# DavidPetrus/ood_object_detection

Hardware: AMD Instinct MI355X
Metric: images/sec, tf_efficientdet_d0 640px bf16 inference + OOD score (DetBenchPredict end-to-end) (higher is better)
Workload: dtype bf16; 1 GPU; tf_efficientdet_d0 640x640 batch=64/GPU C=90, DetBenchPredict: backbone+BiFPN+heads+OOD energy/max-logit+top-k(5000)+decode+hard NMS; global_batch=64, parallelism=image-sharded dp1, no collective, weights=seeded reference init, randomised BN stats, class bias 0, launch=hipgraph, images_in_flight=192

## Files before the change

### ood_object_detection_amd/csrc/common.h

```cpp
#pragma once
#include <hip/hip_runtime.h>
#include <stdint.h>
#include "../../include/effdet_hip.h"

#define EFFDET_OK 0
#define EFFDET_EINVAL (-22)
#define EFFDET_ELAUNCH (-5)

typedef __bf16 bf16_t;
typedef __bf16 bf16x8 __attribute__((ext_vector_type(8)));
typedef float f32x4 __attribute__((ext_vector_type(4)));
typedef unsigned int u32x4 __attribute__((ext_vector_type(4)));

#define DEV __device__ __forceinline__

#define EFFDET_ENTER() (void)hipGetLastError()

extern thread_local int effdet_last_hip_error;
#define EFFDET_DEVICE_ERROR_CODE 0x7EFFDE7
__attribute__((visibility("hidden"))) extern volatile int* effdet_err_host;
__attribute__((visibility("hidden"))) int* effdet_device_error_word();
static inline int effdet_check_launch() {
    hipError_t e = hipGetLastError();
    if (e != hipSuccess) { effdet_last_hip_error = (int)e; return EFFDET_ELAUNCH; }
// ... 7 lines not shown
DEV float fast_silu(float x) { return x * __builtin_amdgcn_rcpf(1.0f + fast_exp(-x)); }
DEV float sigmoid_train(float x) { return __builtin_amdgcn_rcpf(1.0f + __builtin_amdgcn_exp2f(x * -1.4426950408889634f)); }
DEV float silu_train(float x) { return x * sigmoid_train(x); }
DEV float silu_grad(float z) { const float s = sigmoid_train(z); return s * (1.0f + z * (1.0f - s)); }

struct bf16p_t;
template <typename T> struct FastMath { static constexpr bool value = sizeof(T) == 2; };
template <> struct FastMath<bf16p_t> { static constexpr bool value = true; };
template <typename T> DEV float silu_t(float x) {
    if constexpr (FastMath<T>::value) return fast_silu(x); else return silu_f(x);
}
template <typename T> DEV float exp_t(float x) {
    if constexpr (FastMath<T>::value) return fast_exp(x); else return expf(x);
}

typedef float f32x2 __attribute__((ext_vector_type(2)));
DEV f32x4 silu4_scaled(const f32x4 t, const float addc) {
    const f32x2 t0 = {t[0], t[1]}, t1 = {t[2], t[3]};
    const float d00 = __builtin_amdgcn_exp2f(t0[0]) + addc, d01 = __builtin_amdgcn_exp2f(t0[1]) + addc;
    const float d10 = __builtin_amdgcn_exp2f(t1[0]) + addc, d11 = __builtin_amdgcn_exp2f(t1[1]) + addc;
    const f32x2 y0 = t0 * f32x2{__builtin_amdgcn_rcpf(d00), __builtin_amdgcn_rcpf(d01)};
    const f32x2 y1 = t1 * f32x2{__builtin_amdgcn_rcpf(d10), __builtin_amdgcn_rcpf(d11)};
    return f32x4{y0[0], y0[1], y1[0], y1[1]};
}

DEV f32x4 silu4_fast(const f32x4 x) {
    const f32x2 x0 = {x[0], x[1]}, x1 = {x[2], x[3]};
    const f32x2 t0 = x0 * -1.4426950408889634f, t1 = x1 * -1.4426950408889634f;
    const f32x2 d0 = f32x2{__builtin_amdgcn_exp2f(t0[0]), __builtin_amdgcn_exp2f(t0[1])} + 1.0f;
    const f32x2 d1 = f32x2{__builtin_amdgcn_exp2f(t1[0]), __builtin_amdgcn_exp2f(t1[1])} + 1.0f;
    const f32x2 y0 = x0 * f32x2{__builtin_amdgcn_rcpf(d0[0]), __builtin_amdgcn_rcpf(d0[1])};
    const f32x2 y1 = x1 * f32x2{__builtin_amdgcn_rcpf(d1[0]), __builtin_amdgcn_rcpf(d1[1])};
    return f32x4{y0[0], y0[1], y1[0], y1[1]};
}

template <int V> struct IntC { static constexpr int value = V; };

template <typename T> DEV f32x4 bn_silu4(const f32x4 acc, const f32x4 sc, const f32x4 sh) {
    if constexpr (FastMath<T>::value) {
        const f32x2 x0 = f32x2{acc[0], acc[1]} * f32x2{sc[0], sc[1]} + f32x2{sh[0], sh[1]};
        const f32x2 x1 = f32x2{acc[2], acc[3]} * f32x2{sc[2], sc[3]} + f32x2{sh[2], sh[3]};
        const f32x2 t0 = x0 * -1.4426950408889634f, t1 = x1 * -1.4426950408889634f;
        const f32x2 d0 = f32x2{__builtin_amdgcn_exp2f(t0[0]), __builtin_amdgcn_exp2f(t0[1])} + 1.0f;
        const f32x2 d1 = f32x2{__builtin_amdgcn_exp2f(t1[0]), __builtin_amdgcn_exp2f(t1[1])} + 1.0f;
        const f32x2 y0 = x0 * f32x2{__builtin_amdgcn_rcpf(d0[0]), __builtin_amdgcn_rcpf(d0[1])};
        const f32x2 y1 = x1 * f32x2{__builtin_amdgcn_rcpf(d1[0]), __builtin_amdgcn_rcpf(d1[1])};
        return f32x4{y0[0], y0[1], y1[0], y1[1]};
    } else {
        f32x4 y;
#pragma unroll
        for (int r = 0; r < 4; ++r) y[r] = silu_f(acc[r] * sc[r] + sh[r]);
        return y;
    }
}

template <typename T> struct VecTraits;
template <> struct VecTraits<float> { static constexpr int EPC = 4; };
template <> struct VecTraits<bf16_t> { static constexpr int EPC = 8; };

struct F8 { float v[8]; };

template <typename T> DEV F8 load8(const T* p);
template <> DEV F8 load8<float>(const float* p) {
    F8 r;
    const f32x4 a = *reinterpret_cast<const f32x4*>(p);
    const f32x4 b = *reinterpret_cast<const f32x4*>(p + 4);
// ... 211 lines not shown
```

### ood_object_detection_amd/csrc/sepconv.hip

```cpp
#include "common.h"
#include <type_traits>

namespace {

struct SepInput {
    const void* ptr; long long image_stride;
    int H, W; int mode;
    int pad_t, pad_l;
};
struct SepLevel {
    int H, W, tiles_x, tiles_y, tile_begin, affine_row;
    SepInput in[3];
    void* out; long long out_image_stride;
    long long ood_off;
    int in_affine_row;
    void* dw_out; long long dw_out_image_stride;
};
struct SepArgs {
    int nlevels; SepLevel lv[5];
    int n_in, fuse_mode;
    float fw[3]; float fden;
    float fwn[3];
    int vec_ok;
    int out_f32;
    int pre_act, post_act;
    const float* dw_w;
    const void* pw_w;
    const float* scale; const float* shift;
    int F, N;
    int ood_classes, num_anchors;
    float* ood_energy; float* ood_maxlogit; long long ood_image_stride;
    const float* in_scale; const float* in_shift;
    float* stat_partial;
    int tiles_total;
};

constexpr int FC = 64;



template <typename T> struct Raw8 { u32x4 v[sizeof(T) == 2 ? 1 : 2]; };
template <typename T> DEV Raw8<T> load_raw8(const T* p) {
    Raw8<T> r;
    r.v[0] = *reinterpret_cast<const u32x4*>(p);
    if constexpr (sizeof(T) == 4) r.v[1] = *(reinterpret_cast<const u32x4*>(p) + 1);
    return r;
}
template <typename T> DEV F8 unpack8(const Raw8<T>& r) {
    F8 o;
    if constexpr (IsPair<T>::value) {
        return pair_join8(r.v[0], r.v[1]);
    } else if constexpr (sizeof(T) == 2) {
        const bf16x8 a = __builtin_bit_cast(bf16x8, r.v[0]);
#pragma unroll
        for (int e = 0; e < 8; ++e) o.v[e] = (float)a[e];
    } else {
        const f32x4 a = __builtin_bit_cast(f32x4, r.v[0]), b = __builtin_bit_cast(f32x4, r.v[1]);
#pragma unroll
        for (int e = 0; e < 4; ++e) { o.v[e] = a[e]; o.v[4 + e] = b[e]; }
    }
    return o;
}
template <typename T> DEV Raw8<T> pack8(const F8& f) {
    Raw8<T> r;
    if constexpr (IsPair<T>::value) {
        pair_split8(f, r.v[0], r.v[1]);
    } else if constexpr (sizeof(T) == 2) {
        bf16x8 a;
#pragma unroll
        for (int e = 0; e < 8; ++e) a[e] = (bf16_t)f.v[e];
        r.v[0] = __builtin_bit_cast(u32x4, a);
    } else {
        r.v[0] = __builtin_bit_cast(u32x4, f32x4{f.v[0], f.v[1], f.v[2], f.v[3]});
        r.v[1] = __builtin_bit_cast(u32x4, f32x4{f.v[4], f.v[5], f.v[6], f.v[7]});
    }
    return r;
}

template <typename T>
DEV Raw8<T> fetch_input(const T* base, const SepInput& in, int y, int x, int F, int c) {
    if (in.mode != 2) {
        const int sh = in.mode == 1 ? 1 : 0;
        return load_raw8<T>(base + ((y >> sh) * in.W + (x >> sh)) * F + c);
    }
    F8 m = f8_fill(-INFINITY);
#pragma unroll
    for (int ky = 0; ky < 3; ++ky) {
        const int iy = 2 * y + ky - in.pad_t;
        const int iyc = iy < 0 ? 0 : (iy >= in.H ? in.H - 1 : iy);
#pragma unroll
        for (int kx = 0; kx < 3; ++kx) {
            const int ix = 2 * x + kx - in.pad_l;
            const int ixc = ix < 0 ? 0 : (ix >= in.W ? in.W - 1 : ix);
            const F8 v = load8<T>(base + (iyc * in.W + ixc) * F + c);
            const bool inside = iy == iyc && ix == ixc;
#pragma unroll
            for (int e = 0; e < 8; ++e) m.v[e] = fmaxf(m.v[e], inside ? v.v[e] : -INFINITY);
        }
    }
    return pack8<T>(m);
}

template <typename T>
DEV void store_piece(T* dst, const float (&v)[8], int nvalid, bool vec_ok) {
    if constexpr (IsPair<T>::value) {
        typedef unsigned u32x4_a4 __attribute__((ext_vector_type(4), aligned(4)));
        F8 f;
#pragma unroll
        for (int e = 0; e < 8; ++e) f.v[e] = v[e];
        u32x4 hi, lo;
        pair_split8(f, hi, lo);
        if (nvalid >= 8) {
            *reinterpret_cast<u32x4_a4*>(dst) = hi;
            *(reinterpret_cast<u32x4_a4*>(dst) + 1) = lo;
        }
    } else
    if (vec_ok && nvalid >= 8) {
        if constexpr (sizeof(T) == 2) {
            typedef unsigned u32x4_a4 __attribute__((ext_vector_type(4), aligned(4)));
            bf16x8 a;
#pragma unroll
            for (int e = 0; e < 8; ++e) a[e] = (bf16_t)v[e];
            *reinterpret_cast<u32x4_a4*>(dst) = __builtin_bit_cast(u32x4, a);
        } else {
            typedef float f32x4_a4 __attribute__((ext_vector_type(4), aligned(4)));
            *reinterpret_cast<f32x4_a4*>(dst) = f32x4{v[0], v[1], v[2], v[3]};
            *reinterpret_cast<f32x4_a4*>(dst + 4) = f32x4{v[4], v[5], v[6], v[7]};
        }
    } else {
        if constexpr (!IsPair<T>::value) {
#pragma unroll
            for (int e = 0; e < 8; ++e)
                if (e < nvalid) dst[e] = from_f<T>(v[e]);
        }
    }
}

template <typename T, int TH, int TW, int BN, bool OOD, int NTH, int FT, bool META = false, int NIN = 3, bool BST = false>
__global__ __launch_bounds__(NTH, NTH == 512 ? (FT == 64 && !OOD && !META && !IsPair<T>::value ? 8 : 4) : 2) void sepconv_kernel(SepArgs p) {
    constexpr int BM = TH * TW;
    constexpr int HW_ = (TH + 2) * (TW + 2);
    constexpr int NWAVE = NTH / 64;
    constexpr int WPT = BM / (16 * NWAVE);
    constexpr int NT = BN / 16;
    constexpr int NP = NT / 2;
    static_assert(NT % 2 == 0 && WPT >= 1, "tile shape");
    extern __shared__ __attribute__((aligned(16))) char lds[];

    const int F = FT ? FT : p.F, N = p.N;
    const int fbytes = F * (int)sizeof(T);
    constexpr int PB = OpGeom<T>::PIECE, CHB = OpGeom<T>::CHUNK;
    const int nkc = (fbytes + CHB - 1) / CHB;
    const int arow = nkc * CHB + 16;
    constexpr bool MF = IsFast<T>::value && TW == 16 && NTH == 512;
    constexpr int HROW = FC + (MF ? 16 / (int)sizeof(T) : 0);
    constexpr int HALO_BYTES = HW_ * HROW * (int)sizeof(T);
    constexpr bool CP = MF && FT == 64 && !META;
    const int r0 = CP ? (HALO_BYTES > (BM + BN) * arow ? HALO_BYTES : (BM + BN) * arow)
                      : (HALO_BYTES > BN * arow ? HALO_BYTES : BN * arow);
    char* halo = lds;
    char* Wt = CP ? lds + BM * arow : lds;
    char* At = CP ? lds : lds + r0;
    float* dww = reinterpret_cast<float*>(CP ? lds + r0 : At + BM * arow);
    float* cs = dww + 9 * F;

    const int tid = threadIdx.x, lane = tid & 63, wave = tid >> 6;
    const int b = blockIdx.y;
    int li = 0;
#pragma unroll
    for (int q = 1; q < 5; ++q) if (q < p.nlevels && (int)blockIdx.x >= p.lv[q].tile_begin) li = q;
    const SepLevel& L = p.lv[li];
    const int t = blockIdx.x - L.tile_begin;
    const int y0 = (t / L.tiles_x) * TH, x0 = (t % L.tiles_x) * TW;
    const int H = L.H, W = L.W;

    constexpr int DPC = (9 * 128 + NTH - 1) / NTH;
    const bool d_pref = 9 * F <= DPC * NTH;
    float dpre[DPC];
#pragma unroll
    for (int q = 0; q < DPC; ++q) {
        const int i = tid + NTH * q;
        dpre[q] = (d_pref && i < 9 * F) ? p.dw_w[i] : 0.f;
    }
    if (nkc * CHB > fbytes) {
        const int padb = nkc * CHB - fbytes;
        for (int i = tid; i < BM * (padb / 16); i += NTH) {
            const int row = i / (padb / 16), piece = i % (padb / 16);
            *reinterpret_cast<u32x4*>(At + row * arow + fbytes + piece * 16) = u32x4{0u, 0u, 0u, 0u};
        }
    }
    const T* ib[3];
#pragma unroll
    for (int i = 0; i < 3; ++i) {
        const int ii = i < p.n_in ? i : 0;
        ib[i] = reinterpret_cast<const T*>(L.in[ii].ptr) + (long long)b * L.in[ii].image_stride;
    }
    float fwm[3];
#pragma unroll
    for (int i = 0; i < 3; ++i) fwm[i] = i < p.n_in ? ((IsFast<T>::value && p.fuse_mode == 1) ? p.fwn[i] : p.fw[i]) : 0.f;
    const bool divide = !IsFast<T>::value && p.fuse_mode == 1;

    for (int fc0 = 0; fc0 < F; fc0 += FC) {
        const int fcn = (F - fc0) < FC ? (F - fc0) : FC;
        const int fcg = fcn / 8;
        __syncthreads();
        constexpr int HU = NTH == 512 ? ((FT == 64 && !OOD && !META && NIN > 1) ? 1 : ((FT == 0 && NIN > 1) ? 2 : 3)) : 2;
        for (int it0 = tid; it0 < HW_ * fcg; it0 += HU * NTH) {
            Raw8<T> xin[HU][NIN];
            unsigned okm[HU];
#pragma unroll
            for (int u = 0; u < HU; ++u) {
                const int it_ = it0 + NTH * u;
                const int it = it_ < HW_ * fcg ? it_ : HW_ * fcg - 1;
                const int cgh = it % fcg, hp = it / fcg;
                const int y = y0 + hp / (TW + 2) - 1, x = x0 + hp % (TW + 2) - 1;
                const int yc = y < 0 ? 0 : (y >= H ? H - 1 : y), xc = x < 0 ? 0 : (x >= W ? W - 1 : x);
                okm[u] = (it_ < HW_ * fcg && y == yc && x == xc) ? 0xFFFFFFFFu : 0u;
                const int c = fc0 + cgh * 8;
#pragma unroll
                for (int i = 0; i < NIN; ++i) xin[u][i] = fetch_input<T>(ib[i], L.in[i < p.n_in ? i : 0], yc, xc, F, c);
            }
#pragma unroll
            for (int u = 0; u < HU; ++u) {
                const int it = it0 + NTH * u;
                const int cgh = it % fcg, hp = it / fcg;
                const u32x4 km = {okm[u], okm[u], okm[u], okm[u]};
                F8 v = f8_zero();
                {
                    if (p.fuse_mode == 0) {
                        Raw8<T> r0 = xin[u][0];
                        r0.v[0] = r0.v[0] & km;
                        if constexpr (sizeof(T) == 4) r0.v[1] = r0.v[1] & km;
                        v = unpack8<T>(r0);
                    } else {
#pragma unroll
                        for (int i = 0; i < NIN; ++i) {
                            Raw8<T> ri = xin[u][i];
                            ri.v[0] = ri.v[0] & km;
                            if constexpr (sizeof(T) == 4) ri.v[1] = ri.v[1] & km;
                            const F8 xi = unpack8<T>(ri);
                            if (divide) {
#pragma unroll
                                for (int e = 0; e < 8; ++e) v.v[e] += (xi.v[e] * fwm[i]) / p.fden;
                            } else {
#pragma unroll
                                for (int e = 0; e < 8; ++e) v.v[e] = fmaf(xi.v[e], fwm[i], v.v[e]);
                            }
                        }
                    }
                    if constexpr (META) {
                        if (p.in_scale != nullptr) {
                            const F8 is = load8<float>(p.in_scale + (long long)L.in_affine_row * F + fc0 + cgh * 8);
                            const F8 it = load8<float>(p.in_shift + (long long)L.in_affine_row * F + fc0 + cgh * 8);
#pragma unroll
                            for (int e = 0; e < 8; ++e) v.v[e] = okm[u] ? v.v[e] * is.v[e] + it.v[e] : 0.f;
                        }
                    }
                    if (p.pre_act) {
#pragma unroll
                        for (int e = 0; e < 8; ++e) v.v[e] = silu_t<T>(v.v[e]);
                    }
                }
                if (it < HW_ * fcg) store8<T>(reinterpret_cast<T*>(halo) + hp * HROW + cgh * 8, v);
            }
        }
        if (fc0 == 0) {
            if (d_pref) {
#pragma unroll
                for (int q = 0; q < DPC; ++q) {
                    const int i = tid + NTH * q;
                    if (i < 9 * F) dww[i] = dpre[q];
                }
            } else {
                for (int i = tid; i < 9 * F; i += NTH) dww[i] = p.dw_w[i];
            }
        }
        __syncthreads();
        if constexpr (MF) {
            const int frow_ = lane & 15, fp_ = lane >> 4;
            const int j = wave & 3, part = wave >> 2;
            f32x4 keep[CP ? TH / 2 : 1];
            if (16 * j < fcn) {
                const int hi = fp_ >> 1;
                const bool active = (fp_ & 1) == (frow_ >> 3);
                const int dq = (frow_ & 7) >> 1;
                Frag<T> afr[5];
#pragma unroll
                for (int pr = 0; pr < 5; ++pr) {
                    const int t = 2 * pr + hi;
                    const bool on = active && t < 9 && 16 * j + frow_ < fcn;
                    const float wv = on ? dww[(t < 9 ? t : 0) * F + fc0 + 16 * j + frow_] : 0.f;
                    const bf16_t wh = (bf16_t)wv;
                    const unsigned bits = (unsigned)__builtin_bit_cast(unsigned short, wh) << (16 * (frow_ & 1));
// ... 95 lines not shown
            cpre_s = scale ? scale[n_begin + tc] : 1.0f;
            return;
        }
#pragma unroll
        for (int q = 0; q < WPC; ++q) {
            const int i = tid + NTH * q;
            u32x4 v = {0u, 0u, 0u, 0u};
            if (i < BN * ppr) {
                const int co = i / ppr, piece = i % ppr;
                if (co < n_count && piece * 16 < fbytes)
                    v = *reinterpret_cast<const u32x4*>(reinterpret_cast<const char*>(p.pw_w) +
                                                        (long long)(n_begin + co) * fbytes + piece * 16);
            }
            wpre[q] = v;
        }
        if (tid < BN) {
            cpre_s = (scale && tid < n_count) ? scale[n_begin + tid] : 1.0f;
            cpre_t = tid < n_count ? shift[n_begin + tid] : 0.0f;
        }
    };
    if (prefetch) w_fetch(0);

    int pix_off[WPT];
    bool pix_in[WPT];
#pragma unroll
    for (int i = 0; i < WPT; ++i) {
        const int prow = 16 * WPT * wave + 16 * i + frow;
        const int y = y0 + prow / TW, x = x0 + prow % TW;
        pix_in[i] = y < H && x < W;
        pix_off[i] = (y * W + x) * N;
    }
    __amdgpu_buffer_rsrc_t ors, ers, mrs;
    constexpr int OB = IsPair<T>::value ? 4 : 2;
    if constexpr (BST) {
        ors = __builtin_amdgcn_make_buffer_rsrc(reinterpret_cast<char*>(L.out) + (long long)b * L.out_image_stride * OB, 0, H * W * N * OB, 0x00020000);
        ers = __builtin_amdgcn_make_buffer_rsrc(reinterpret_cast<char*>(p.ood_energy + (long long)b * p.ood_image_stride + L.ood_off), 0,
                                                H * W * p.num_anchors * 4, 0x00020000);
        mrs = __builtin_amdgcn_make_buffer_rsrc(reinterpret_cast<char*>(p.ood_maxlogit + (long long)b * p.ood_image_stride + L.ood_off), 0,
                                                H * W * p.num_anchors * 4, 0x00020000);
    }
    int o128[BST ? WPT : 1][NP], otail[BST ? WPT : 1][3], oscore[BST ? WPT : 1];
    const int jstar = C / 32;
    if constexpr (BST) {
        constexpr int OOB = 0x7FFFFFF0;
#pragma unroll
        for (int i = 0; i < WPT; ++i) {
            const int sb = pix_off[i] * OB + fpiece * 8 * OB;
#pragma unroll
            for (int J = 0; J < NP; ++J) o128[i][J] = (pix_in[i] && C - (32 * J + 8 * fpiece) >= 8) ? sb + 32 * OB * J : OOB;
            const int nvt = C - (32 * jstar + 8 * fpiece);
#pragma unroll
            for (int d = 0; d < 3; ++d)
                otail[i][d] = (pix_in[i] && nvt > 0 && nvt < 8 && 2 * d < nvt) ? sb + 32 * OB * jstar + 2 * OB * d : OOB;
            oscore[i] = (pix_in[i] && fpiece == 0) ? (pix_off[i] / N) * p.num_anchors * 4 : OOB;
        }
    }
    float run_m[WPT], run_s[WPT];
    constexpr float LOG2E = 1.4426950408889634f;

    for (int ch = 0; ch < nchunks; ++ch) {
        int n_begin, n_count;
        chunk_range(ch, n_begin, n_count);
        __syncthreads();
        if constexpr (META) {
            if (ch == 0 && L.dw_out != nullptr) {
                T* dwo = reinterpret_cast<T*>(L.dw_out) + (long long)b * L.dw_out_image_stride;
// ... 10 lines not shown
        if (BST) {
#pragma unroll
            for (int q = 0; q < WPC; ++q) {
                const int i = tid + NTH * q < BN * ppr ? tid + NTH * q : BN * ppr - 1;
                const int co = i / ppr, piece = i % ppr;
                const unsigned keep = (co < n_count && piece * 16 < fbytes) ? 0xFFFFFFFFu : 0u;
                *reinterpret_cast<u32x4*>(Wt + lds_row(co) * arow + piece * 16) = wpre[q] & u32x4{keep, keep, keep, keep};
            }
            if (tid < BN) cs[BN + tid] = tid < n_count ? cpre_t : -INFINITY;
        } else if (prefetch) {
#pragma unroll
            for (int q = 0; q < WPC; ++q) {
                const int i = tid + NTH * q;
                if (i < BN * ppr) *reinterpret_cast<u32x4*>(Wt + lds_row(i / ppr) * arow + (i % ppr) * 16) = wpre[q];
            }
            if (tid < BN) { cs[tid] = cpre_s; cs[BN + tid] = cpre_t; }
        } else {
            for (int i = tid; i < BN * ppr; i += NTH) {
                const int co = i / ppr, piece = i % ppr;
                u32x4 v = {0u, 0u, 0u, 0u};
                if (co < n_count && piece * 16 < fbytes)
                    v = *reinterpret_cast<const u32x4*>(reinterpret_cast<const char*>(p.pw_w) +
                                                        (long long)(n_begin + co) * fbytes + piece * 16);
                *reinterpret_cast<u32x4*>(Wt + lds_row(co) * arow + piece * 16) = v;
            }
            if (tid < BN) {
                cs[tid] = (scale && tid < n_count) ? scale[n_begin + tid] : 1.0f;
                cs[BN + tid] = tid < n_count ? shift[n_begin + tid] : 0.0f;
            }
        }
        __syncthreads();
        if (prefetch && ch + 1 < nchunks) w_fetch(ch + 1);

        const int njp = (n_count + 31) / 32;
        f32x4 acc[WPT][NT];
#pragma unroll
        for (int i = 0; i < WPT; ++i)
#pragma unroll
            for (int j = 0; j < NT; ++j) acc[i][j] = f32x4{0.f, 0.f, 0.f, 0.f};
        for (int kc = 0; kc < nkc; ++kc) {
            Frag<T> xb[WPT];
#pragma unroll
            for (int i = 0; i < WPT; ++i)
                xb[i] = ld_frag<T>(At + (16 * WPT * wave + 16 * i + frow) * arow + kc * CHB + fpiece * PB);
#pragma unroll
            for (int j = 0; j < NT; ++j) {
                if (j < 2 * njp) {
                    const Frag<T> wf = ld_frag<T>(Wt + (16 * j + frow) * arow + kc * CHB + fpiece * PB);
#pragma unroll
                    for (int i = 0; i < WPT; ++i) mma_chunk(wf, xb[i], acc[i][j]);
                }
            }
        }

        if constexpr (BST) {
            constexpr float LN2 = 0.6931471805599453f;
            const int so = n_begin * OB, sa = ch * 4;
#pragma unroll
            for (int i = 0; i < WPT; ++i) {
                f32x4 v[NT];
#pragma unroll
                for (int J = 0; J < NP; ++J) {
                    const int cb = 32 * J + 8 * fpiece;
                    v[2 * J] = acc[i][2 * J] + *reinterpret_cast<const f32x4*>(cs + BN + cb);
                    v[2 * J + 1] = acc[i][2 * J + 1] + *reinterpret_cast<const f32x4*>(cs + BN + cb + 4);
                }
                if constexpr (IsPair<T>::value) {
// ... 12 lines not shown
                    u32x4 pk[NP];
#pragma unroll
                    for (int J = 0; J < NP; ++J) {
                        const bf16x8 a8 = {(bf16_t)v[2 * J][0], (bf16_t)v[2 * J][1], (bf16_t)v[2 * J][2], (bf16_t)v[2 * J][3],
                                           (bf16_t)v[2 * J + 1][0], (bf16_t)v[2 * J + 1][1], (bf16_t)v[2 * J + 1][2], (bf16_t)v[2 * J + 1][3]};
                        pk[J] = __builtin_bit_cast(u32x4, a8);
                        __builtin_amdgcn_raw_buffer_store_b128(pk[J], ors, o128[i][J], so, 0);
                    }
                    u32x4 pt = pk[0];
#pragma unroll
                    for (int J = 1; J < NP; ++J) pt = jstar == J ? pk[J] : pt;
#pragma unroll
                    for (int d = 0; d < 3; ++d) __builtin_amdgcn_raw_buffer_store_b32(pt[d], ors, otail[i][d], so, 0);
                }
                float m = -INFINITY;
#pragma unroll
                for (int j = 0; j < NT; ++j) m = fmaxf(m, fmaxf(fmaxf(v[j][0], v[j][1]), fmaxf(v[j][2], v[j][3])));
                m = fmaxf(m, __shfl_xor(m, 16, 64));
                m = fmaxf(m, __shfl_xor(m, 32, 64));
                const float tl = m * LOG2E;
                f32x2 s2 = {0.f, 0.f};
#pragma unroll
                for (int j = 0; j < NT; ++j) {
                    const f32x2 e0 = f32x2{v[j][0], v[j][1]} * LOG2E - tl, e1 = f32x2{v[j][2], v[j][3]} * LOG2E - tl;
                    s2 += f32x2{__builtin_amdgcn_exp2f(e0[0]), __builtin_amdgcn_exp2f(e0[1])};
                    s2 += f32x2{__builtin_amdgcn_exp2f(e1[0]), __builtin_amdgcn_exp2f(e1[1])};
                }
                float ssum = s2[0] + s2[1];
                ssum += __shfl_xor(ssum, 16, 64);
                ssum += __shfl_xor(ssum, 32, 64);
                const float energy = IsPair<T>::value ? -(m + logf(ssum)) : -(m + LN2 * __builtin_amdgcn_logf(ssum));
                __builtin_amdgcn_raw_buffer_store_b32(__builtin_bit_cast(unsigned, energy), ers, oscore[i], sa, 0);
                __builtin_amdgcn_raw_buffer_store_b32(__builtin_bit_cast(unsigned, m), mrs, oscore[i], sa, 0);
            }
            continue;
        }
        float stq[META ? WPT : 1][META ? NP : 1][8];
        if constexpr (META) {
#pragma unroll
            for (int i = 0; i < WPT; ++i)
#pragma unroll
                for (int J = 0; J < NP; ++J)
#pragma unroll
                    for (int e = 0; e < 8; ++e) stq[i][J][e] = 0.f;
        }
#pragma unroll
        for (int i = 0; i < WPT; ++i) {
            float m = -INFINITY, ssum = 0.f;
            float vals[NP][8];
#pragma unroll
            for (int J = 0; J < NP; ++J) {
                if (J < njp) {
                    const int cb = 32 * J + 8 * fpiece;
                    const f32x4 t0 = *reinterpret_cast<const f32x4*>(cs + BN + cb);
                    const f32x4 t1 = *reinterpret_cast<const f32x4*>(cs + BN + cb + 4);
                    f32x4 s0 = {1.f, 1.f, 1.f, 1.f}, s1 = {1.f, 1.f, 1.f, 1.f};
                    if (scale) {
                        s0 = *reinterpret_cast<const f32x4*>(cs + cb);
                        s1 = *reinterpret_cast<const f32x4*>(cs + cb + 4);
                    }
#pragma unroll
                    for (int r = 0; r < 4; ++r) {
                        float a0 = fmaf(acc[i][2 * J][r], s0[r], t0[r]);
                        float a1 = fmaf(acc[i][2 * J + 1][r], s1[r], t1[r]);
                        if (p.post_act) { a0 = silu_t<T>(a0); a1 = silu_t<T>(a1); }
                        vals[J][r] = a0; vals[J][4 + r] = a1;
// ... 108 lines not shown
                        for (int o = 1; o < 16; o <<= 1) { a += __shfl_xor(a, o, 64); q += __shfl_xor(q, o, 64); }
                        if (frow == 0) { sst[(wave * 2 + 0) * BN + 32 * J + 8 * fpiece + e] = a; sst[(wave * 2 + 1) * BN + 32 * J + 8 * fpiece + e] = q; }
                    }
                __syncthreads();
                if (tid < 2 * BN) {
                    const int which = tid / BN, n = tid % BN;
                    float tot = 0.f;
                    for (int w = 0; w < NWAVE; ++w) tot += sst[(w * 2 + which) * BN + n];
                    if (n < n_count) {
                        float* row = p.stat_partial + (((long long)b * p.tiles_total + blockIdx.x) * 3) * N + n_begin + n;
                        row[(1 + which) * (long long)N] = tot;
                        if (which == 0) row[0] = piv[n];
                    }
                }
            }
        }
    }
}

template <typename T, int TH, int TW, int BN>
size_t sep_lds_bytes(int F, bool cp = false) {
    constexpr int BM = TH * TW;
    constexpr int HW_ = (TH + 2) * (TW + 2);
    const int nkc = (F * (int)sizeof(T) + OpGeom<T>::CHUNK - 1) / OpGeom<T>::CHUNK;
    const int arow = nkc * OpGeom<T>::CHUNK + 16;
    const size_t halo = (size_t)HW_ * (FC + (IsFast<T>::value && TW == 16 ? 16 / (int)sizeof(T) : 0)) * sizeof(T);
    const size_t wt = (size_t)BN * arow;
    if (cp) return (halo > wt + (size_t)BM * arow ? halo : wt + (size_t)BM * arow) + (size_t)9 * F * 4 + (size_t)2 * BN * 4;
    return (halo > wt ? halo : wt) + (size_t)BM * arow + (size_t)9 * F * 4 + (size_t)2 * BN * 4;
}

struct SepPlan { int v[EFFDET_SEPCONV_PLAN_INTS]; };

template <typename T, int TH, int TW, int BN, bool OOD, int NTH, int FT, bool META = false, int NIN = 3, bool BST = false>
int launch_sep(hipStream_t st, SepArgs& a, int B, SepPlan* plan = nullptr) {
    int tiles = 0;
    for (int i = 0; i < a.nlevels; ++i) {
        a.lv[i].tiles_x = (a.lv[i].W + TW - 1) / TW;
        a.lv[i].tiles_y = (a.lv[i].H + TH - 1) / TH;
        a.lv[i].tile_begin = tiles;
        tiles += a.lv[i].tiles_x * a.lv[i].tiles_y;
    }
    const size_t lds = sep_lds_bytes<T, TH, TW, BN>(a.F, IsFast<T>::value && TW == 16 && NTH == 512 && FT == 64 && !META) + (META ? (size_t)(NTH / 64) * 2 * BN * 4 : 0);
    if (lds > 160 * 1024) return EFFDET_EINVAL;
    a.tiles_total = tiles;
    if (plan) {
        constexpr int DPC = (9 * 128 + NTH - 1) / NTH, CHB = OpGeom<T>::CHUNK;
        constexpr int WPC = (BN * (CHB / 8) + NTH - 1) / NTH;
        const int nkc = (a.F * (int)sizeof(T) + CHB - 1) / CHB, ppr = nkc * (CHB / 16);
        const int subs = OOD ? (a.ood_classes + BN - 1) / BN : 1;
        const int v[EFFDET_SEPCONV_PLAN_INTS] = {
            IsPair<T>::value ? 2 : (sizeof(T) == 2 ? 1 : 0), TH, TW, NTH, FT, BN, OOD ? 1 : 0, BST ? 1 : 0, NIN, META ? 1 : 0,
            subs, OOD ? a.num_anchors * subs : (a.N + BN - 1) / BN, tiles, (int)lds,
            9 * a.F <= DPC * NTH ? 1 : 0, BN * ppr <= NTH * WPC ? 1 : 0, a.out_f32, a.vec_ok};
        for (int i = 0; i < EFFDET_SEPCONV_PLAN_INTS; ++i) plan->v[i] = v[i];
        return EFFDET_OK;
    }
    auto kern = sepconv_kernel<T, TH, TW, BN, OOD, NTH, FT, META, NIN, BST>;
    if (lds > 64 * 1024) {
        static bool attr_done = false;
        if (!attr_done) {
            if (hipFuncSetAttribute(reinterpret_cast<const void*>(kern), hipFuncAttributeMaxDynamicSharedMemorySize, 160 * 1024) != hipSuccess)
                return EFFDET_ELAUNCH;
            attr_done = true;
        }
    }
    hipLaunchKernelGGL(kern, dim3(tiles, B), dim3(NTH), lds, st, a);
    return effdet_check_launch();
}

constexpr int BST_TH = 8;
template <typename T, int TH, int TW, int NTH, int FT>
int dispatch_sep_f(hipStream_t st, SepArgs& a, int B, SepPlan* plan = nullptr) {
    if (a.ood_classes > 0) {
        if constexpr (FT == 0) {
            if (sep_lds_bytes<T, TH, TW, 96>(a.F) > 160 * 1024) return launch_sep<T, TH, TW, 64, true, NTH, FT>(st, a, B, plan);
        }
        if constexpr (IsPair<T>::value && NTH == 512) {
            if (a.out_f32 && a.ood_classes % 2 == 0 && a.ood_classes <= 96 && a.F <= 64 && a.scale == nullptr && !a.post_act)
                return launch_sep<T, BST_TH, TW, 96, true, NTH, FT, false, 3, true>(st, a, B, plan);
        }
        if constexpr (sizeof(T) == 2 && NTH == 512) {
            if (a.vec_ok && !a.out_f32 && a.ood_classes % 2 == 0 && a.ood_classes <= 96 && a.F <= 64 && a.scale == nullptr && !a.post_act)
                return launch_sep<T, BST_TH, TW, 96, true, NTH, FT, false, 3, true>(st, a, B, plan);
        }
        return launch_sep<T, TH, TW, 96, true, NTH, FT>(st, a, B, plan);
    }
    if (FT == 64 && a.n_in == 1) return launch_sep<T, TH, TW, 64, false, NTH, FT, false, 1>(st, a, B, plan);
    return launch_sep<T, TH, TW, 64, false, NTH, FT>(st, a, B, plan);
}

template <typename T, int TH, int TW, int NTH>
int dispatch_sep(hipStream_t st, SepArgs& a, int B, SepPlan* plan = nullptr) {
    switch (a.F) {
        case 64:  return dispatch_sep_f<T, TH, TW, NTH, 64>(st, a, B, plan);
        case 88:  return dispatch_sep_f<T, TH, TW, NTH, 88>(st, a, B, plan);
        case 112: return dispatch_sep_f<T, TH, TW, NTH, 112>(st, a, B, plan);
        case 160: return dispatch_sep_f<T, TH, TW, NTH, 160>(st, a, B, plan);
        case 224: return dispatch_sep_f<T, TH, TW, NTH, 224>(st, a, B, plan);
        default:  return dispatch_sep_f<T, TH, TW, NTH, 0>(st, a, B, plan);
    }
}

template <int FT>
int dispatch_sep_pair_8x8(hipStream_t st, SepArgs& a, int B, SepPlan* plan = nullptr) {
    if (a.ood_classes > 0) {
        if constexpr (FT == 0) {
            if (sep_lds_bytes<bf16p_t, 8, 8, 96>(a.F) > 160 * 1024) return launch_sep<bf16p_t, 8, 8, 64, true, 256, 0>(st, a, B, plan);
        }
        return launch_sep<bf16p_t, 8, 8, 96, true, 256, FT>(st, a, B, plan);
    }
    return launch_sep<bf16p_t, 8, 8, 64, false, 256, FT>(st, a, B, plan);
}

}

namespace {
struct MetaExtra {
    const float* in_scale; const float* in_shift; const int* in_affine_row;
// ... 41 lines not shown
    const int* level_hw,
    int n_in,
    const void* const* in_ptr,
    const long long* in_image_stride,
    const int* in_hw,
    const int* in_mode,
    int fuse_mode, const float* fuse_w, float fuse_den, int pre_act,
    const float* dw_w, const void* pw_w, const float* scale, const float* shift,
    const int* affine_row,
    int post_act, int F, int N,
    void* const* out_ptr, const long long* out_image_stride,
    int ood_classes, int num_anchors, float* ood_energy, float* ood_maxlogit,
    long long ood_image_stride, const long long* ood_level_off) {
    if (!level_hw || !in_ptr || !in_image_stride || !in_hw || !in_mode || !dw_w || !pw_w || !shift || !affine_row ||
        !out_ptr || !out_image_stride) return EFFDET_EINVAL;
    const int sym = take_pad_flag(dtype);
    int out_f32 = 0;
    if (sep_check_shape(dtype, out_f32, meta != nullptr, B, nlevels, level_hw, n_in, fuse_mode, F, N, ood_classes, num_anchors) != EFFDET_OK)
        return EFFDET_EINVAL;
    if (fuse_mode != 0 && !fuse_w) return EFFDET_EINVAL;
    if (ood_classes > 0 && (!ood_energy || !ood_maxlogit || !ood_level_off)) return EFFDET_EINVAL;
    SepArgs a;
    a.nlevels = nlevels; a.n_in = n_in; a.fuse_mode = fuse_mode; a.fden = fuse_den;
    for (int i = 0; i < 3; ++i) a.fw[i] = (fuse_mode != 0 && i < n_in) ? fuse_w[i] : 0.f;
    for (int i = 0; i < 3; ++i) a.fwn[i] = fuse_mode == 1 ? a.fw[i] / fuse_den : a.fw[i];
    const size_t esz = (dtype == 0 || out_f32) ? 4 : 2;
    a.out_f32 = out_f32;
    a.vec_ok = sep_rows_dword_aligned(N, ood_classes, esz);
    a.pre_act = pre_act; a.post_act = post_act; a.dw_w = dw_w; a.pw_w = pw_w; a.scale = scale; a.shift = shift;
    a.F = F; a.N = N; a.ood_classes = ood_classes > 0 ? ood_classes : 0; a.num_anchors = num_anchors;
    a.ood_energy = ood_energy; a.ood_maxlogit = ood_maxlogit; a.ood_image_stride = ood_image_stride;
    a.in_scale = meta ? meta->in_scale : nullptr; a.in_shift = meta ? meta->in_shift : nullptr;
    a.stat_partial = meta ? meta->stat_partial : nullptr; a.tiles_total = 0;
    if (meta && ((meta->in_scale != nullptr) != (meta->in_shift != nullptr) || (meta->in_scale && !meta->in_affine_row))) return EFFDET_EINVAL;
    for (int l = 0; l < nlevels; ++l) {
        SepLevel& L = a.lv[l];
        L.in_affine_row = (meta && meta->in_affine_row) ? meta->in_affine_row[l] : 0;
        L.dw_out = (meta && meta->dw_out) ? meta->dw_out[l] : nullptr;
        L.dw_out_image_stride = (meta && meta->dw_out_image_stride) ? meta->dw_out_image_stride[l] : 0;
        if (L.dw_out && reinterpret_cast<uintptr_t>(L.dw_out) % 16) return EFFDET_EINVAL;
        L.H = level_hw[2 * l]; L.W = level_hw[2 * l + 1];
        L.affine_row = affine_row[l];
        L.out = out_ptr[l]; L.out_image_stride = out_image_stride[l];
        L.ood_off = (ood_classes > 0) ? ood_level_off[l] : 0;
        if (!L.out) return EFFDET_EINVAL;
        if (reinterpret_cast<uintptr_t>(L.out) % 16 || ((size_t)L.out_image_stride * esz) % 4) a.vec_ok = 0;
        for (int i = 0; i < n_in; ++i) {
            SepInput& I = L.in[i];
            I.ptr = in_ptr[l * n_in + i]; I.image_stride = in_image_stride[l * n_in + i];
            I.H = in_hw[(l * n_in + i) * 2]; I.W = in_hw[(l * n_in + i) * 2 + 1];
            I.mode = in_mode[l * n_in + i];
            I.pad_t = I.pad_l = 0;
            if (!I.ptr) return EFFDET_EINVAL;
            if (I.mode == 0) { if (I.H != L.H || I.W != L.W) return EFFDET_EINVAL; }
            else if (I.mode == 1) { if (I.H * 2 != L.H || I.W * 2 != L.W) return EFFDET_EINVAL; }
            else if (I.mode == 2) {
                if (same_out(I.H, 2) != L.H || same_out(I.W, 2) != L.W) return EFFDET_EINVAL;
                I.pad_t = pad_before(I.H, 3, 2, sym); I.pad_l = pad_before(I.W, 3, 2, sym);
            } else return EFFDET_EINVAL;
        }
    }
    if (dtype == 2) {
        for (int l = 0; l < nlevels; ++l) {
            if (!out_f32 && (reinterpret_cast<uintptr_t>(a.lv[l].out) % 16 || a.lv[l].out_image_stride % 4)) return EFFDET_EINVAL;
            for (int i = 0; i < n_in; ++i)
                if (reinterpret_cast<uintptr_t>(a.lv[l].in[i].ptr) % 16 || a.lv[l].in[i].image_stride % 4) return EFFDET_EINVAL;
        }
    }
    return sep_dispatch(meta != nullptr, dtype, reinterpret_cast<hipStream_t>(stream), a, B, nullptr);
}

extern "C" int effdet_sepconv_fused(
    void* stream, int dtype, int B, int nlevels, const int* level_hw, int n_in,
    const void* const* in_ptr, const long long* in_image_stride, const int* in_hw, const int* in_mode,
    int fuse_mode, const float* fuse_w, float fuse_den, int pre_act,
    const float* dw_w, const void* pw_w, const float* scale, const float* shift, const int* affine_row,
    int post_act, int F, int N, void* const* out_ptr, const long long* out_image_stride,
    int ood_classes, int num_anchors, float* ood_energy, float* ood_maxlogit,
    long long ood_image_stride, const long long* ood_level_off) {
    EFFDET_ENTER();
    return sepconv_common(nullptr, stream, dtype, B, nlevels, level_hw, n_in, in_ptr, in_image_stride, in_hw, in_mode,
                          fuse_mode, fuse_w, fuse_den, pre_act, dw_w, pw_w, scale, shift, affine_row, post_act, F, N,
                          out_ptr, out_image_stride, ood_classes, num_anchors, ood_energy, ood_maxlogit, ood_image_stride, ood_level_off);
}

extern "C" int effdet_sepconv_meta(
    void* stream, int dtype, int B, int nlevels, const int* level_hw,
    const void* const* in_ptr, const long long* in_image_stride,
    const float* in_scale, const float* in_shift, const int* in_affine_row, int pre_act,
    const float* dw_w, const void* pw_w, const float* bias, int F, int N,
    void* const* out_ptr, const long long* out_image_stride,
    float* stat_partial, void* const* dw_out, const long long* dw_out_image_stride) {
    EFFDET_ENTER();
// ... 101 lines not shown
```

Measured before the change: 17130 images/sec.

## Add trimmed sepconv kernel variants specialised by live inputs and epilogue

Adds TRIM template variants of the bf16 F=64 separable-conv kernel. They load only the live fused inputs, copy raw halo data when there is a single input with no fusion or pre-activation, and skip the max-pool bounds masking when the padding geometry makes it unnecessary. A simplified epilogue applies BN (optionally followed by SiLU) and writes bf16x8 with buffer stores over fixed 64-wide N tiles. The host checks which pooling and padding cases are safe and dispatches to these variants. The aim is fewer registers, less halo-building ALU work and a cheaper store path, at the cost of more template instantiations and correctness that depends on the padding checks.

```diff
diff --git a/ood_object_detection_amd/csrc/common.h b/ood_object_detection_amd/csrc/common.h
--- a/ood_object_detection_amd/csrc/common.h
+++ b/ood_object_detection_amd/csrc/common.h
@@ -63,6 +63,13 @@
     const f32x2 y0 = x0 * f32x2{__builtin_amdgcn_rcpf(d0[0]), __builtin_amdgcn_rcpf(d0[1])};
     const f32x2 y1 = x1 * f32x2{__builtin_amdgcn_rcpf(d1[0]), __builtin_amdgcn_rcpf(d1[1])};
     return f32x4{y0[0], y0[1], y1[0], y1[1]};
+}
+
+DEV f32x2 fma2(const f32x2 a, const f32x2 b, const f32x2 c) { return __builtin_elementwise_fma(a, b, c); }
+DEV f32x4 fma4(const f32x4 a, const f32x4 b, const f32x4 c) {
+    const f32x2 r0 = fma2(f32x2{a[0], a[1]}, f32x2{b[0], b[1]}, f32x2{c[0], c[1]});
+    const f32x2 r1 = fma2(f32x2{a[2], a[3]}, f32x2{b[2], b[3]}, f32x2{c[2], c[3]});
+    return f32x4{r0[0], r0[1], r1[0], r1[1]};
 }
 
 template <int V> struct IntC { static constexpr int value = V; };
diff --git a/ood_object_detection_amd/csrc/sepconv.hip b/ood_object_detection_amd/csrc/sepconv.hip
--- a/ood_object_detection_amd/csrc/sepconv.hip
+++ b/ood_object_detection_amd/csrc/sepconv.hip
@@ -33,6 +33,7 @@
     const float* in_scale; const float* in_shift;
     float* stat_partial;
     int tiles_total;
+    int trim_ok;
 };
 
 constexpr int FC = 64;
@@ -77,9 +78,9 @@
     return r;
 }
 
-template <typename T>
+template <typename T, int POOL = 0>
 DEV Raw8<T> fetch_input(const T* base, const SepInput& in, int y, int x, int F, int c) {
-    if (in.mode != 2) {
+    if (POOL == 2 || in.mode != 2) {
         const int sh = in.mode == 1 ? 1 : 0;
         return load_raw8<T>(base + ((y >> sh) * in.W + (x >> sh)) * F + c);
     }
@@ -93,7 +94,7 @@
             const int ix = 2 * x + kx - in.pad_l;
             const int ixc = ix < 0 ? 0 : (ix >= in.W ? in.W - 1 : ix);
             const F8 v = load8<T>(base + (iyc * in.W + ixc) * F + c);
-            const bool inside = iy == iyc && ix == ixc;
+            const bool inside = POOL == 1 || (iy == iyc && ix == ixc);
 #pragma unroll
             for (int e = 0; e < 8; ++e) m.v[e] = fmaxf(m.v[e], inside ? v.v[e] : -INFINITY);
         }
@@ -136,7 +137,8 @@
     }
 }
 
-template <typename T, int TH, int TW, int BN, bool OOD, int NTH, int FT, bool META = false, int NIN = 3, bool BST = false>
+constexpr int TRIM_RAWH = 4, TRIM_SLE = 8, TRIM_POST = 16, TRIM_DIRECT = 32;
+template <typename T, int TH, int TW, int BN, bool OOD, int NTH, int FT, bool META = false, int NIN = 3, bool BST = false, int TRIM = 0>
 __global__ __launch_bounds__(NTH, NTH == 512 ? (FT == 64 && !OOD && !META && !IsPair<T>::value ? 8 : 4) : 2) void sepconv_kernel(SepArgs p) {
     constexpr int BM = TH * TW;
     constexpr int HW_ = (TH + 2) * (TW + 2);
@@ -145,6 +147,10 @@
     constexpr int NT = BN / 16;
     constexpr int NP = NT / 2;
     static_assert(NT % 2 == 0 && WPT >= 1, "tile shape");
+    constexpr int LIVE = TRIM ? (TRIM & 3) : NIN;
+    constexpr bool PK = TRIM != 0, RAWH = (TRIM & TRIM_RAWH) != 0, SLE = (TRIM & TRIM_SLE) != 0, POST = (TRIM & TRIM_POST) != 0;
+    static_assert(!TRIM || (sizeof(T) == 2 && !IsPair<T>::value && FT == 64 && NTH == 512 && !META), "TRIM forms: bf16, F = 64");
+    static_assert(LIVE >= 1 && LIVE <= NIN && (!RAWH || LIVE == 1) && (!SLE || BN == 64) && (!POST || SLE) && (!TRIM || !OOD), "TRIM bits");
     extern __shared__ __attribute__((aligned(16))) char lds[];
 
     const int F = FT ? FT : p.F, N = p.N;
@@ -189,15 +195,15 @@
             *reinterpret_cast<u32x4*>(At + row * arow + fbytes + piece * 16) = u32x4{0u, 0u, 0u, 0u};
         }
     }
-    const T* ib[3];
-#pragma unroll
-    for (int i = 0; i < 3; ++i) {
+    const T* ib[LIVE];
+#pragma unroll
+    for (int i = 0; i < LIVE; ++i) {
         const int ii = i < p.n_in ? i : 0;
         ib[i] = reinterpret_cast<const T*>(L.in[ii].ptr) + (long long)b * L.in[ii].image_stride;
     }
-    float fwm[3];
-#pragma unroll
-    for (int i = 0; i < 3; ++i) fwm[i] = i < p.n_in ? ((IsFast<T>::value && p.fuse_mode == 1) ? p.fwn[i] : p.fw[i]) : 0.f;
+    float fwm[LIVE];
+#pragma unroll
+    for (int i = 0; i < LIVE; ++i) fwm[i] = i < p.n_in ? ((IsFast<T>::value && p.fuse_mode == 1) ? p.fwn[i] : p.fw[i]) : 0.f;
     const bool divide = !IsFast<T>::value && p.fuse_mode == 1;
 
     for (int fc0 = 0; fc0 < F; fc0 += FC) {
@@ -206,7 +212,7 @@
         __syncthreads();
         constexpr int HU = NTH == 512 ? ((FT == 64 && !OOD && !META && NIN > 1) ? 1 : ((FT == 0 && NIN > 1) ? 2 : 3)) : 2;
         for (int it0 = tid; it0 < HW_ * fcg; it0 += HU * NTH) {
-            Raw8<T> xin[HU][NIN];
+            Raw8<T> xin[HU][LIVE];
             unsigned okm[HU];
 #pragma unroll
             for (int u = 0; u < HU; ++u) {
@@ -218,13 +224,18 @@
                 okm[u] = (it_ < HW_ * fcg && y == yc && x == xc) ? 0xFFFFFFFFu : 0u;
                 const int c = fc0 + cgh * 8;
 #pragma unroll
-                for (int i = 0; i < NIN; ++i) xin[u][i] = fetch_input<T>(ib[i], L.in[i < p.n_in ? i : 0], yc, xc, F, c);
+                for (int i = 0; i < LIVE; ++i) xin[u][i] = fetch_input<T, (TRIM & TRIM_DIRECT) ? 2 : (TRIM ? 1 : 0)>(ib[i], L.in[i < p.n_in ? i : 0], yc, xc, F, c);
             }
 #pragma unroll
             for (int u = 0; u < HU; ++u) {
                 const int it = it0 + NTH * u;
                 const int cgh = it % fcg, hp = it / fcg;
                 const u32x4 km = {okm[u], okm[u], okm[u], okm[u]};
+                if constexpr (RAWH) {
+                    if (it < HW_ * fcg)
+                        *reinterpret_cast<u32x4*>(reinterpret_cast<T*>(halo) + hp * HROW + cgh * 8) = xin[u][0].v[0] & km;
+                    continue;
+                }
                 F8 v = f8_zero();
                 {
                     if (p.fuse_mode == 0) {
@@ -234,11 +245,19 @@
                         v = unpack8<T>(r0);
                     } else {
 #pragma unroll
-                        for (int i = 0; i < NIN; ++i) {
+                        for (int i = 0; i < LIVE; ++i) {
                             Raw8<T> ri = xin[u][i];
                             ri.v[0] = ri.v[0] & km;
                             if constexpr (sizeof(T) == 4) ri.v[1] = ri.v[1] & km;
                             const F8 xi = unpack8<T>(ri);
+                            if constexpr (PK) {
+                                const f32x2 w2 = {fwm[i], fwm[i]};
+#pragma unroll
+                                for (int e = 0; e < 8; e += 2) {
+                                    const f32x2 r = fma2(f32x2{xi.v[e], xi.v[e + 1]}, w2, f32x2{v.v[e], v.v[e + 1]});
+                                    v.v[e] = r[0]; v.v[e + 1] = r[1];
+                                }
+                            } else
                             if (divide) {
 #pragma unroll
                                 for (int e = 0; e < 8; ++e) v.v[e] += (xi.v[e] * fwm[i]) / p.fden;
@@ -257,8 +276,14 @@
                         }
                     }
                     if (p.pre_act) {
-#pragma unroll
-                        for (int e = 0; e < 8; ++e) v.v[e] = silu_t<T>(v.v[e]);
+                        if constexpr (PK) {
+                            const f32x4 a = silu4_fast(f32x4{v.v[0], v.v[1], v.v[2], v.v[3]}), c = silu4_fast(f32x4{v.v[4], v.v[5], v.v[6], v.v[7]});
+#pragma unroll
+                            for (int e = 0; e < 4; ++e) { v.v[e] = a[e]; v.v[4 + e] = c[e]; }
+                        } else {
+#pragma unroll
+                            for (int e = 0; e < 8; ++e) v.v[e] = silu_t<T>(v.v[e]);
+                        }
                     }
                 }
                 if (it < HW_ * fcg) store8<T>(reinterpret_cast<T*>(halo) + hp * HROW + cgh * 8, v);
@@ -420,6 +445,12 @@
     }
     __amdgpu_buffer_rsrc_t ors, ers, mrs;
     constexpr int OB = IsPair<T>::value ? 4 : 2;
+    int osle[SLE ? WPT : 1];
+    if constexpr (SLE) {
+        ors = __builtin_amdgcn_make_buffer_rsrc(reinterpret_cast<char*>(L.out) + (long long)b * L.out_image_stride * 2, 0, H * W * N * 2, 0x00020000);
+#pragma unroll
+        for (int i = 0; i < WPT; ++i) osle[i] = pix_in[i] ? pix_off[i] * 2 + fpiece * 16 : 0x7FFFFF00;
+    }
     if constexpr (BST) {
         ors = __builtin_amdgcn_make_buffer_rsrc(reinterpret_cast<char*>(L.out) + (long long)b * L.out_image_stride * OB, 0, H * W * N * OB, 0x00020000);
         ers = __builtin_amdgcn_make_buffer_rsrc(reinterpret_cast<char*>(p.ood_energy + (long long)b * p.ood_image_stride + L.ood_off), 0,
@@ -496,7 +527,7 @@
         __syncthreads();
         if (prefetch && ch + 1 < nchunks) w_fetch(ch + 1);
 
-        const int njp = (n_count + 31) / 32;
+        const int njp = SLE ? NP : (n_count + 31) / 32;
         f32x4 acc[WPT][NT];
 #pragma unroll
         for (int i = 0; i < WPT; ++i)
@@ -575,6 +606,23 @@
                 const float energy = IsPair<T>::value ? -(m + logf(ssum)) : -(m + LN2 * __builtin_amdgcn_logf(ssum));
                 __builtin_amdgcn_raw_buffer_store_b32(__builtin_bit_cast(unsigned, energy), ers, oscore[i], sa, 0);
                 __builtin_amdgcn_raw_buffer_store_b32(__builtin_bit_cast(unsigned, m), mrs, oscore[i], sa, 0);
+            }
+            continue;
+        }
+        if constexpr (SLE) {
+            const int so = n_begin * 2;
+#pragma unroll
+            for (int J = 0; J < NP; ++J) {
+                const int cb = 32 * J + 8 * fpiece;
+                const f32x4 s0 = *reinterpret_cast<const f32x4*>(cs + cb), s1 = *reinterpret_cast<const f32x4*>(cs + cb + 4);
+                const f32x4 t0 = *reinterpret_cast<const f32x4*>(cs + BN + cb), t1 = *reinterpret_cast<const f32x4*>(cs + BN + cb + 4);
+#pragma unroll
+                for (int i = 0; i < WPT; ++i) {
+                    const f32x4 a0 = POST ? bn_silu4<T>(acc[i][2 * J], s0, t0) : fma4(acc[i][2 * J], s0, t0);
+                    const f32x4 a1 = POST ? bn_silu4<T>(acc[i][2 * J + 1], s1, t1) : fma4(acc[i][2 * J + 1], s1, t1);
+                    const bf16x8 a8 = {(bf16_t)a0[0], (bf16_t)a0[1], (bf16_t)a0[2], (bf16_t)a0[3], (bf16_t)a1[0], (bf16_t)a1[1], (bf16_t)a1[2], (bf16_t)a1[3]};
+                    __builtin_amdgcn_raw_buffer_store_b128(__builtin_bit_cast(u32x4, a8), ors, osle[i] + 64 * J, so, 0);
+                }
             }
             continue;
         }
@@ -749,7 +797,7 @@
 
 struct SepPlan { int v[EFFDET_SEPCONV_PLAN_INTS]; };
 
-template <typename T, int TH, int TW, int BN, bool OOD, int NTH, int FT, bool META = false, int NIN = 3, bool BST = false>
+template <typename T, int TH, int TW, int BN, bool OOD, int NTH, int FT, bool META = false, int NIN = 3, bool BST = false, int TRIM = 0>
 int launch_sep(hipStream_t st, SepArgs& a, int B, SepPlan* plan = nullptr) {
     int tiles = 0;
     for (int i = 0; i < a.nlevels; ++i) {
@@ -773,7 +821,7 @@
         for (int i = 0; i < EFFDET_SEPCONV_PLAN_INTS; ++i) plan->v[i] = v[i];
         return EFFDET_OK;
     }
-    auto kern = sepconv_kernel<T, TH, TW, BN, OOD, NTH, FT, META, NIN, BST>;
+    auto kern = sepconv_kernel<T, TH, TW, BN, OOD, NTH, FT, META, NIN, BST, TRIM>;
     if (lds > 64 * 1024) {
         static bool attr_done = false;
         if (!attr_done) {
@@ -802,6 +850,22 @@
                 return launch_sep<T, BST_TH, TW, 96, true, NTH, FT, false, 3, true>(st, a, B, plan);
         }
         return launch_sep<T, TH, TW, 96, true, NTH, FT>(st, a, B, plan);
+    }
+    if constexpr (sizeof(T) == 2 && !IsPair<T>::value && NTH == 512 && FT == 64) {
+        bool sle = a.N % 64 == 0 && a.vec_ok && !a.out_f32;
+        for (int l = 0; l < a.nlevels; ++l) sle = sle && (long long)a.lv[l].H * a.lv[l].W * a.N * 2 < (1ll << 30);
+        const bool direct = (a.trim_ok & 2) != 0;
+        if (a.n_in == 1 && a.fuse_mode == 0 && !a.pre_act && direct) {
+            constexpr int R = 1 | TRIM_RAWH | TRIM_DIRECT;
+            if (sle && a.post_act) return launch_sep<T, TH, TW, 64, false, NTH, FT, false, 1, false, R | TRIM_SLE | TRIM_POST>(st, a, B, plan);
+            if (sle) return launch_sep<T, TH, TW, 64, false, NTH, FT, false, 1, false, R | TRIM_SLE>(st, a, B, plan);
+            return launch_sep<T, TH, TW, 64, false, NTH, FT, false, 1, false, R>(st, a, B, plan);
+        }
+        if (a.n_in >= 2 && a.fuse_mode != 0 && sle && !a.post_act && (a.trim_ok & 1)) {
+            if (a.n_in == 2 && direct) return launch_sep<T, TH, TW, 64, false, NTH, FT, false, 3, false, 2 | TRIM_SLE | TRIM_DIRECT>(st, a, B, plan);
+            if (a.n_in == 2) return launch_sep<T, TH, TW, 64, false, NTH, FT, false, 3, false, 2 | TRIM_SLE>(st, a, B, plan);
+            return launch_sep<T, TH, TW, 64, false, NTH, FT, false, 3, false, 3 | TRIM_SLE>(st, a, B, plan);
+        }
     }
     if (FT == 64 && a.n_in == 1) return launch_sep<T, TH, TW, 64, false, NTH, FT, false, 1>(st, a, B, plan);
     return launch_sep<T, TH, TW, 64, false, NTH, FT>(st, a, B, plan);
@@ -909,6 +973,7 @@
     a.ood_energy = ood_energy; a.ood_maxlogit = ood_maxlogit; a.ood_image_stride = ood_image_stride;
     a.in_scale = meta ? meta->in_scale : nullptr; a.in_shift = meta ? meta->in_shift : nullptr;
     a.stat_partial = meta ? meta->stat_partial : nullptr; a.tiles_total = 0;
+    a.trim_ok = 3;
     if (meta && ((meta->in_scale != nullptr) != (meta->in_shift != nullptr) || (meta->in_scale && !meta->in_affine_row))) return EFFDET_EINVAL;
     for (int l = 0; l < nlevels; ++l) {
         SepLevel& L = a.lv[l];
@@ -934,8 +999,12 @@
             else if (I.mode == 2) {
                 if (same_out(I.H, 2) != L.H || same_out(I.W, 2) != L.W) return EFFDET_EINVAL;
                 I.pad_t = pad_before(I.H, 3, 2, sym); I.pad_l = pad_before(I.W, 3, 2, sym);
+                a.trim_ok &= ~2;
+                if (!(I.pad_t >= 0 && I.pad_t <= 1 && I.pad_l >= 0 && I.pad_l <= 1 &&
+                      2 * (L.H - 1) - I.pad_t <= I.H - 1 && 2 * (L.W - 1) - I.pad_l <= I.W - 1)) a.trim_ok = 0;
             } else return EFFDET_EINVAL;
         }
+        for (int i = n_in; i < 3; ++i) L.in[i] = SepInput{nullptr, 0, 0, 0, 0, 0, 0};
     }
     if (dtype == 2) {
         for (int l = 0; l < nlevels; ++l) {
```

New measurement: 16950 images/sec. 0.99x the previous value.
